# arrufat/zignal

Measured on NVIDIA H100. Metric: Mpixels/sec Gaussian-blur 8K RGBA f32, higher is better.
Workload: dtype f32

## Files before the change

### zignal_b200/csrc/zb_conv_fused.cu

```cuda
#include "zb_conv.h"
#include "zb_device.cuh"
#include "zb_shard.h"
#include "zb_tma.cuh"

namespace zb {

namespace {

constexpr int TW = 256;
constexpr int CHUNK = 8;
constexpr int G = TW / 8 + 2;
constexpr int STAGE_BYTES = G * CHUNK * 128;
constexpr int RING_ROWS = 24;
constexpr int RING_ROW_BYTES = TW * 16;
constexpr int RING_BYTES = RING_ROWS * RING_ROW_BYTES;
constexpr int NTHREADS = 256;
constexpr int MAX_HALF = 8;
constexpr int MAXK = 2 * MAX_HALF + 1;
constexpr int STAGES = 2;
constexpr int SMEM_BYTES = STAGES * STAGE_BYTES + RING_BYTES + 64 + 1024;

struct FusedParams {
    float kx[MAXK];
    float ky[MAXK];
    const float4* src;
    float4* dst;
    unsigned long long src_pitch_px, dst_pitch_px;
    int rows, cols, border;
    int ngroups;
    int n_strips;
    int n_units;
    int strip_lo, strip_hi;
    int n_segs, seg_chunks, seg_extra;
    int e_segs, e_chunks, e_extra;
    int row0, row1;
    int fix_rows;
    int fix_left;
    int fix_right;
    int tma_row_off;
    int edge_fast;
    int lsrc[8];
    int rsrc[8];
};

struct ShardParams {
    const float4* up_rows;
    const float4* down_rows;
    unsigned long long up_pitch_px, down_pitch_px;
    int half;
    ShardLink link;
};

template <bool ROTATE>
__device__ __forceinline__ void unit_at(const FusedParams& p, int u, int& strip, int& ra, int& rb) {
    const int n_inner = p.strip_hi - p.strip_lo;
    int seg, chunks, extra;
    if (u < p.n_segs * n_inner) {
        seg = u / n_inner;
        strip = p.strip_lo + (u - seg * n_inner);
        if constexpr (ROTATE) seg = seg + 1 == p.n_segs ? 0 : seg + 1;
        chunks = p.seg_chunks;
        extra = p.seg_extra;
    } else {
        const int n_edge = p.n_strips - n_inner;
        u -= p.n_segs * n_inner;
        seg = u / n_edge;
        const int e = u - seg * n_edge;
        strip = e < p.strip_lo ? e : e - p.strip_lo + p.strip_hi;
        chunks = p.e_chunks;
        extra = p.e_extra;
    }
    ra = p.row0 + (seg * chunks + min(seg, extra)) * CHUNK;
    rb = min(ra + (chunks + (seg < extra ? 1 : 0)) * CHUNK, p.row1);
}

template <bool EXACT>
__device__ __forceinline__ void mac4(float4& acc, const float4& v, float k) {
    if constexpr (EXACT) {
        acc.x = __fadd_rn(acc.x, __fmul_rn(v.x, k));
        acc.y = __fadd_rn(acc.y, __fmul_rn(v.y, k));
        acc.z = __fadd_rn(acc.z, __fmul_rn(v.z, k));
        acc.w = __fadd_rn(acc.w, __fmul_rn(v.w, k));
    } else {
        acc.x = fmaf(v.x, k, acc.x);
        acc.y = fmaf(v.y, k, acc.y);
        acc.z = fmaf(v.z, k, acc.z);
        acc.w = fmaf(v.w, k, acc.w);
    }
}

template <bool SHARD>
__device__ __noinline__ void fixup_stage(uint32_t stage, int y0, int xs0, bool fix_x, bool fix_rows, const FusedParams& p,
                                         int nb_lo, int nb_hi) {
    const int xlimit = p.ngroups * 8;
    auto stage_addr = [&](int rr, int xx) {
        const uint32_t line = (uint32_t)(rr * G + (xx >> 3));
        return stage + line * 128 + ((((uint32_t)xx & 7u) ^ (line & 7u)) << 4);
    };
    if (fix_x && p.edge_fast) {
        fix_x = false;
        if (threadIdx.x < 128) {
            const int side = threadIdx.x >> 6, rr = (threadIdx.x >> 3) & 7, e = threadIdx.x & 7;
            const int y = y0 + rr;
            bool row_ok = y >= 0 && y < p.rows;
            if constexpr (SHARD) row_ok = row_ok || (y < 0 && y >= nb_lo) || (y >= p.rows && y < nb_hi);
            const bool edge = side == 0 ? xs0 < 0 : xs0 + G * 8 > p.cols;
            if (row_ok && edge) {
                const int s_dst = side == 0 ? e : p.cols - xs0 + e;
                const int s_src = side == 0 ? p.lsrc[e] : p.rsrc[e] - xs0;
                if (s_dst < G * 8) sts128(stage_addr(rr, s_dst), lds128(stage_addr(rr, s_src)));
            }
        }
    }
    if (fix_x) {
        const int nleft = xs0 < 0 ? min(-xs0, G * 8) : 0;
        const int r0 = max(0, xlimit - xs0);
        const int r1 = min(G * 8, p.cols - xs0 + MAX_HALF);
        const int per_row = nleft + max(0, r1 - r0);
        for (int idx = threadIdx.x; idx < CHUNK * per_row; idx += NTHREADS) {
            const int rr = idx / per_row, e = idx - rr * per_row;
            const int xx = e < nleft ? e : r0 + (e - nleft);
            const int y = y0 + rr, x = xs0 + xx;
            const float4* rowp = p.src + (long long)y * (long long)p.src_pitch_px;
            if (y < 0 || y >= p.rows) {
                if constexpr (SHARD) {
                    if (y < nb_lo || y >= nb_hi) continue;
                } else {
                    continue;
                }
            }
            const int rx = resolve_index(x, p.cols, p.border);
            float4 v = make_float4(0.f, 0.f, 0.f, 0.f);
            if (rx >= 0) {
                const int sx = rx - xs0;
                if (rx < xlimit && sx >= 0 && sx < G * 8) v = lds128(stage_addr(rr, sx));
                else v = __ldg(rowp + rx);
            }
            sts128(stage_addr(rr, xx), v);
        }
    }
    if (fix_rows) {
        for (int idx = threadIdx.x; idx < CHUNK * G * 8; idx += NTHREADS) {
            const int rr = idx / (G * 8);
            const int xx = idx - rr * (G * 8);
            const int y = y0 + rr, x = xs0 + xx;
            if (y >= 0 && y < p.rows) continue;
            if constexpr (SHARD) {
                if (y >= nb_lo && y < nb_hi) continue;
            }
            const int ry = resolve_index(y, p.rows, p.border);
            const int rx = resolve_index(x, p.cols, p.border);
            float4 v = make_float4(0.f, 0.f, 0.f, 0.f);
            if (ry >= 0 && rx >= 0) v = __ldg(p.src + (size_t)ry * p.src_pitch_px + rx);
            sts128(stage_addr(rr, xx), v);
        }
    }
}

template <int HALF, bool EXACT, int SLOT>
__device__ __forceinline__ void v_pass(uint32_t v_col, const FusedParams& p, float4* out, bool col_ok, int rows_left) {
    constexpr int K = 2 * HALF + 1;
    constexpr int NLOAD = CHUNK + 2 * HALF;
    float4 acc[8];
#pragma unroll
    for (int o = 0; o < 8; ++o) acc[o] = make_float4(0.f, 0.f, 0.f, 0.f);
#pragma unroll
    for (int j = 0; j < NLOAD; ++j) {
        const int sr = (SLOT * CHUNK + 8 - HALF + j) % RING_ROWS;
        const float4 v = lds128(v_col + (uint32_t)(sr * RING_ROW_BYTES));
#pragma unroll
        for (int o = 0; o < 8; ++o) {
            const int ti = j - o;
            if (ti >= 0 && ti < K) mac4<EXACT>(acc[o], v, p.ky[ti]);
        }
    }
    if (col_ok) {
#pragma unroll
        for (int o = 0; o < 8; ++o)
            if (o < rows_left) __stcs(out + (size_t)o * p.dst_pitch_px, acc[o]);
    }
}

template <int HALF, bool EXACT, bool SHARD>
__device__ __forceinline__ uint32_t fused_units(const CUtensorMap& tmap, const FusedParams& p, unsigned nbr, int k_begin, int k_end, uint32_t count0) {
    constexpr int K = 2 * HALF + 1;
    constexpr int NLOAD = CHUNK + 2 * HALF;
    extern __shared__ unsigned char smem_raw[];
    const uint32_t smem0 = (smem_u32(smem_raw) + 1023u) & ~1023u;
    const uint32_t ring = smem0 + STAGES * STAGE_BYTES;
    const uint32_t bar0 = ring + RING_BYTES;

    const int tid = threadIdx.x;
    const long long u_first = (long long)blockIdx.x + (long long)k_begin * gridDim.x;
    const long long u_last = (long long)blockIdx.x + (long long)k_end * gridDim.x;
    const int n_units = (int)min((long long)p.n_units, u_last);
    if (u_first >= n_units) return count0;
    auto touches_neighbour = [&](int y) { return ((nbr & 1u) && y < 0) || ((nbr & 2u) && y + CHUNK > p.rows); };

    int pu = (int)u_first, pi = 0;
    uint32_t pcount = count0;
    auto produce = [&]() {
        if (pu >= n_units) return;
        int strip, ra, rb;
        unit_at<SHARD>(p, pu, strip, ra, rb);
        const int n_in = (rb - ra + CHUNK - 1) / CHUNK + 2;
        const uint32_t st = pcount % STAGES;
        const int y = ra - CHUNK + CHUNK * pi;
        fence_proxy_async();
        mbar_arrive_expect_tx(bar0 + 8 * st, STAGE_BYTES);
        tma_load_3d(smem0 + st * STAGE_BYTES, &tmap, 0, strip * (TW / 8) - 1, y + p.tma_row_off, bar0 + 8 * st);
        ++pcount;
        if (++pi == n_in) { pi = 0; pu += gridDim.x; }
    };
    if (tid == 0)
        for (int i = 0; i < STAGES; ++i) produce();

    const int ht = tid & 31, hr = tid >> 5;
    const int vx = tid;
    const uint32_t v_col = ring + (uint32_t)(vx >> 3) * 128u + ((((uint32_t)vx & 7u) ^ (((uint32_t)vx >> 3) & 7u)) << 4);
    const uint32_t h_ring_col = ring + (uint32_t)ht * 128u;
    const uint32_t h_key = (uint32_t)ht & 7u;

    uint32_t ccount = count0;

    for (int unit = (int)u_first; unit < n_units; unit += gridDim.x) {
        int strip, ra, rb;
        unit_at<SHARD>(p, unit, strip, ra, rb);
        const int x0 = strip * TW;
        const int n_out = (rb - ra + CHUNK - 1) / CHUNK;
        const int n_in = n_out + 2;
        const int g0 = x0 / 8 - 1;

        for (int i = 0; i < n_in; ++i, ++ccount) {
            const uint32_t st = ccount % STAGES;
            const uint32_t stage = smem0 + st * STAGE_BYTES;
            while (!mbar_try_wait(bar0 + 8 * st, (ccount / STAGES) & 1u)) {}
            const int y0 = ra - CHUNK + CHUNK * i;
            bool fix_r = p.fix_rows && (y0 < 0 || y0 + CHUNK > p.rows);
            if constexpr (SHARD) {
                if (touches_neighbour(y0)) fix_r = false;
            }
            const bool fix_x = (p.fix_left && g0 < 0) || (p.fix_right && (g0 + G) * 8 > p.ngroups * 8);
            if (fix_r || fix_x) {
                fixup_stage<SHARD>(stage, y0, g0 * 8, fix_x, fix_r, p, (nbr & 1u) ? INT_MIN : 0, (nbr & 2u) ? INT_MAX : p.rows);
                __syncthreads();
            }

            {
                const uint32_t line0 = (uint32_t)(hr * G + ht);
                uint32_t lbase[3];
#pragma unroll
                for (int l = 0; l < 3; ++l) lbase[l] = stage + (line0 + l) * 128u + (((line0 + l) & 7u) << 4);
                const uint32_t rrow = h_ring_col + (uint32_t)(((i % 3) * CHUNK + hr) * RING_ROW_BYTES);
                float4 acc[8];
#pragma unroll
                for (int o = 0; o < 8; ++o) acc[o] = make_float4(0.f, 0.f, 0.f, 0.f);
#pragma unroll
                for (int j = 0; j < NLOAD; ++j) {
                    const int pidx = 8 - HALF + j;
                    const float4 v = lds128(lbase[pidx >> 3] ^ (((uint32_t)pidx & 7u) << 4));
#pragma unroll
                    for (int o = 0; o < 8; ++o) {
                        const int ti = j - o;
                        if (ti >= 0 && ti < K) mac4<EXACT>(acc[o], v, p.kx[ti]);
                    }
                }
#pragma unroll
                for (int o = 0; o < 8; ++o) sts128(rrow + ((((uint32_t)o) ^ h_key) << 4), acc[o]);
            }
            __syncthreads();

            if (tid == 0) produce();

            if (i >= 2) {
                const int c = i - 2;
                const int x = x0 + vx;
                const int yb = ra + CHUNK * c;
                float4* out = p.dst + (size_t)yb * p.dst_pitch_px + x;
                const bool col_ok = x < p.cols;
                switch (c % 3) {
                    case 0: v_pass<HALF, EXACT, 0>(v_col, p, out, col_ok, rb - yb); break;
                    case 1: v_pass<HALF, EXACT, 1>(v_col, p, out, col_ok, rb - yb); break;
                    default: v_pass<HALF, EXACT, 2>(v_col, p, out, col_ok, rb - yb); break;
                }
            }
            __syncthreads();
        }
    }
    return ccount;
}

template <int HALF, bool EXACT, bool SHARD>
__device__ __forceinline__ void fused_sep_rgbaf32_body(const CUtensorMap& tmap, const FusedParams& p, const ShardParams* sp) {
    extern __shared__ unsigned char smem_raw[];
    const uint32_t smem0 = (smem_u32(smem_raw) + 1023u) & ~1023u;
    const uint32_t bar0 = smem0 + STAGES * STAGE_BYTES + RING_BYTES;
    const int tid = threadIdx.x;
    if (tid == 0) {
        asm volatile("prefetch.tensormap [%0];" ::"l"(&tmap) : "memory");
        for (int i = 0; i < STAGES; ++i) mbar_init(bar0 + 8 * i, 1);
        fence_barrier_init();
    }
    if constexpr (!SHARD) {
        __syncthreads();
        fused_units<HALF, EXACT, false>(tmap, p, 0u, 0, INT_MAX / 2048, 0u);
    } else {
        ShardCtrl* me = sp->link.self;
        const unsigned long long epoch = sp->link.epoch;
        const unsigned nbr = (sp->up_rows ? 1u : 0u) | (sp->down_rows ? 2u : 0u);
        const int per_side = sp->half * p.cols;
        const int total = (sp->up_rows ? per_side : 0) + (sp->down_rows ? per_side : 0);
        constexpr int BATCH = 12;
        const int rem = p.n_units % (int)gridDim.x;
        const int n_copiers = (int)gridDim.x - rem;
        const int ci = (int)blockIdx.x - rem;
        const bool copier = ci >= 0 && (long long)ci * NTHREADS * BATCH < total;
        if (tid == 0) {
            if (blockIdx.x == 0) {
                me->dbg[0] = global_timer_ns();
                if (sp->link.up) st_release_sys(&sp->link.up->ready_from[1], epoch);
                if (sp->link.down) st_release_sys(&sp->link.down->ready_from[0], epoch);
            }
            if (copier) {
                if (sp->up_rows) shard_wait_ge(&me->ready_from[0], epoch, me);
                if (sp->down_rows) shard_wait_ge(&me->ready_from[1], epoch, me);
                if (ci == 0) me->dbg[1] = global_timer_ns();
            }
        }
        __syncthreads();
        if (copier) {
            for (int base = ci * NTHREADS * BATCH; base < total; base += n_copiers * NTHREADS * BATCH) {
                float4 v[BATCH];
                float4* dstp[BATCH];
    #pragma unroll
                for (int k = 0; k < BATCH; ++k) {
                    int e = base + k * NTHREADS + tid;
                    dstp[k] = nullptr;
                    if (e < total) {
                        const bool upper = sp->up_rows && e < per_side;
                        if (!upper && sp->up_rows) e -= per_side;
                        const int r = e / p.cols, x = e - r * p.cols;
                        if (upper) {
                            v[k] = *(sp->up_rows + (size_t)r * sp->up_pitch_px + x);
                            dstp[k] = const_cast<float4*>(p.src) + (long long)(r - sp->half) * (long long)p.src_pitch_px + x;
                        } else {
                            v[k] = *(sp->down_rows + (size_t)r * sp->down_pitch_px + x);
                            dstp[k] = const_cast<float4*>(p.src) + (long long)(p.rows + r) * (long long)p.src_pitch_px + x;
                        }
                    }
                }
    #pragma unroll
                for (int k = 0; k < BATCH; ++k)
                    if (dstp[k]) *dstp[k] = v[k];
            }
            asm volatile("fence.proxy.async;" ::: "memory");
            __syncthreads();
        }
        if (tid == 0) {
            __threadfence();
            if (atomicAdd(&me->halo_reads[0], 1u) == gridDim.x - 1u) {
                me->halo_reads[0] = 0;
                me->dbg[2] = global_timer_ns();
                __threadfence();
                st_release_sys(&me->halo_landed, epoch);
                if (sp->up_rows) st_release_sys(&sp->link.up->done_from[1], epoch);
                if (sp->down_rows) st_release_sys(&sp->link.down->done_from[0], epoch);
            }
        }
        const long long first_halo_unit = (long long)max(0, p.n_segs - 2) * p.n_strips;
        const int k_split = first_halo_unit <= (long long)blockIdx.x ? 0 : (int)((first_halo_unit - blockIdx.x + gridDim.x - 1) / gridDim.x);
        const uint32_t count = fused_units<HALF, EXACT, true>(tmap, p, nbr, 0, k_split, 0u);
        if ((long long)blockIdx.x + (long long)k_split * gridDim.x < (long long)p.n_units) {
            if (tid == 0) {
                shard_wait_ge(&me->halo_landed, epoch, me);
                asm volatile("fence.proxy.async;" ::: "memory");
            }
            __syncthreads();
            fused_units<HALF, EXACT, true>(tmap, p, nbr, k_split, INT_MAX / 2048, count);
        }
        if (tid == 0) {
            ShardCtrl* me = sp->link.self;
            __threadfence();
            if (atomicAdd(&me->exit_ticket, 1u) == gridDim.x - 1u) {
                me->exit_ticket = 0;
                me->dbg[3] = global_timer_ns();
                if (sp->link.up) shard_wait_ge(&me->done_from[0], sp->link.epoch, me);
                if (sp->link.down) shard_wait_ge(&me->done_from[1], sp->link.epoch, me);
                me->dbg[4] = global_timer_ns();
            }
        }
    }
}


template <int HALF, bool EXACT>
__global__ void __launch_bounds__(NTHREADS, 1)
fused_sep_rgbaf32_kernel(const __grid_constant__ CUtensorMap tmap, const __grid_constant__ FusedParams p) {
    fused_sep_rgbaf32_body<HALF, EXACT, false>(tmap, p, nullptr);
}

template <int HALF, bool EXACT>
__global__ void __launch_bounds__(NTHREADS, 1)
fused_sep_rgbaf32_shard_kernel(const __grid_constant__ CUtensorMap tmap, const __grid_constant__ FusedParams p,
                               const __grid_constant__ ShardParams sp) {
    fused_sep_rgbaf32_body<HALF, EXACT, true>(tmap, p, &sp);
}

template <int HALF>
int launch_fused(const CUtensorMap& tmap, const FusedParams& p, const ShardParams* sp, int grid, bool exact, cudaStream_t s) {
    if (sp) {
        auto k = exact ? fused_sep_rgbaf32_shard_kernel<HALF, true> : fused_sep_rgbaf32_shard_kernel<HALF, false>;
        ZB_CUDA(cudaFuncSetAttribute(k, cudaFuncAttributeMaxDynamicSharedMemorySize, SMEM_BYTES));
        k<<<grid, NTHREADS, SMEM_BYTES, s>>>(tmap, p, *sp);
    } else {
        auto k = exact ? fused_sep_rgbaf32_kernel<HALF, true> : fused_sep_rgbaf32_kernel<HALF, false>;
        ZB_CUDA(cudaFuncSetAttribute(k, cudaFuncAttributeMaxDynamicSharedMemorySize, SMEM_BYTES));
        k<<<grid, NTHREADS, SMEM_BYTES, s>>>(tmap, p);
    }
    ZB_LAUNCHED();
    return ZB_OK;
}

int launch_half(int half, const CUtensorMap& tmap, const FusedParams& p, const ShardParams* sp, int grid, bool exact, cudaStream_t s) {
    switch (half) {
        case 1: return launch_fused<1>(tmap, p, sp, grid, exact, s);
        case 2: return launch_fused<2>(tmap, p, sp, grid, exact, s);
        case 3: return launch_fused<3>(tmap, p, sp, grid, exact, s);
        case 4: return launch_fused<4>(tmap, p, sp, grid, exact, s);
        case 5: return launch_fused<5>(tmap, p, sp, grid, exact, s);
        case 6: return launch_fused<6>(tmap, p, sp, grid, exact, s);
        case 7: return launch_fused<7>(tmap, p, sp, grid, exact, s);
        case 8: return launch_fused<8>(tmap, p, sp, grid, exact, s);
    }
    return ZB_ERR_UNSUPPORTED;
}

}

static int encode_block_map(EncodeTiledFn encode, CUtensorMap& tmap, void* data, int ngroups, int rows, uint64_t stride_px) {
    const cuuint64_t gdim[3] = {32, (cuuint64_t)ngroups, (cuuint64_t)rows};
    const cuuint64_t gstr[2] = {128, (cuuint64_t)stride_px * 16};
    const cuuint32_t box[3] = {32, (cuuint32_t)G, (cuuint32_t)CHUNK};
    const cuuint32_t estr[3] = {1, 1, 1};
    CUresult cr = encode(&tmap, CU_TENSOR_MAP_DATA_TYPE_FLOAT32, 3, data, gdim, gstr, box, estr, CU_TENSOR_MAP_INTERLEAVE_NONE,
                         CU_TENSOR_MAP_SWIZZLE_128B, CU_TENSOR_MAP_L2_PROMOTION_L2_256B, CU_TENSOR_MAP_FLOAT_OOB_FILL_NONE);
    if (cr != CUDA_SUCCESS) {
        snprintf(t_last_error, sizeof(t_last_error), "cuTensorMapEncodeTiled failed: %d", (int)cr);
        return ZB_ERR_UNSUPPORTED;
    }
    return ZB_OK;
}

constexpr long long EDGE_COST_NUM = 5, EDGE_COST_DEN = 4;

static void plan_units(int nrows, int sm_count, FusedParams& p) {
    const long long chunks = (nrows + CHUNK - 1) / CHUNK;
    const long long max_segs = chunks / 8 < 1 ? 1 : (chunks / 8 < sm_count ? chunks / 8 : sm_count);
    const long long n_inner = p.strip_hi - p.strip_lo, n_edge = p.n_strips - n_inner;
    auto steps = [&](long long segs) { return (chunks + segs - 1) / segs + 2; };
    long long best_cost = -1, best_units = 0, best_s = 1, best_e = 1;
    for (long long s = 1; s <= max_segs; ++s) {
        const long long waves = (s * p.n_strips + sm_count - 1) / sm_count;
        long long e = s;
        if (n_edge > 0) {
            long long e_max = (waves * sm_count - s * n_inner) / n_edge;
            if (e_max > max_segs) e_max = max_segs;
            while (e < e_max && EDGE_COST_NUM * steps(e) > EDGE_COST_DEN * steps(s)) ++e;
        }
        const long long inner = n_inner > 0 ? EDGE_COST_DEN * steps(s) : 0, edge = n_edge > 0 ? EDGE_COST_NUM * steps(e) : 0;
        const long long cost = waves * (inner > edge ? inner : edge), units = s * n_inner + e * n_edge;
        if (best_cost < 0 || cost < best_cost || (cost == best_cost && units < best_units)) {
            best_cost = cost;
            best_units = units;
            best_s = s;
            best_e = e;
        }
    }
    p.n_units = (int)best_units;
    p.n_segs = (int)best_s;
    p.seg_chunks = (int)(chunks / best_s);
    p.seg_extra = (int)(chunks % best_s);
    p.e_segs = (int)best_e;
    p.e_chunks = (int)(chunks / best_e);
    p.e_extra = (int)(chunks % best_e);
}

static int fused_prepare(const zb_image* src, zb_image* dst, const float* kx, int nx, const float* ky, int ny, int border, int row0, int row1,
                         bool bands, FusedParams& p, CUtensorMap& tmap, int& grid, int& half_out, EncodeTiledFn& encode) {
    const int half_x = nx / 2, half_y = ny / 2;
    const int half = half_x > half_y ? half_x : half_y;
    if (half < 1 || half > MAX_HALF) return ZB_ERR_UNSUPPORTED;
    if (src->cols < 16 || src->rows < 16) return ZB_ERR_UNSUPPORTED;
    if (images_overlap(src, dst, 16)) return ZB_ERR_UNSUPPORTED;
    if (((uintptr_t)src->data & 15u) || ((uintptr_t)dst->data & 15u)) return ZB_ERR_UNSUPPORTED;
    for (int i = 0; i < nx; ++i) if (fabsf(kx[i]) < 1e-10f) return ZB_ERR_UNSUPPORTED;
    for (int i = 0; i < ny; ++i) if (fabsf(ky[i]) < 1e-10f) return ZB_ERR_UNSUPPORTED;
    encode = encode_tiled_fn();
    if (!encode) return ZB_ERR_UNSUPPORTED;
    DeviceInfo di;
    int rc = device_info(&di);
    if (rc) return rc;
    if (di.smem_optin < (size_t)SMEM_BYTES) return ZB_ERR_UNSUPPORTED;

    memset(&p, 0, sizeof(p));
    for (int i = 0; i < nx; ++i) p.kx[i + (half - half_x)] = kx[i];
    for (int i = 0; i < ny; ++i) p.ky[i + (half - half_y)] = ky[i];
    p.src = (const float4*)src->data;
    p.dst = (float4*)dst->data;
    p.src_pitch_px = src->stride;
    p.dst_pitch_px = dst->stride;
    p.rows = (int)src->rows;
    p.cols = (int)src->cols;
    p.border = border;
    p.ngroups = p.cols / 8;
    p.n_strips = (p.cols + TW - 1) / TW;
    p.row0 = row0 < 0 ? 0 : row0;
    p.row1 = (row1 < 0 || row1 > p.rows) ? p.rows : row1;
    if (p.row1 <= p.row0) { grid = 0; return ZB_OK; }
    const int nrows = p.row1 - p.row0;
    p.fix_rows = border != ZB_BORDER_ZERO;
    p.fix_left = border != ZB_BORDER_ZERO;
    p.fix_right = (border != ZB_BORDER_ZERO) || (p.cols % 8 != 0);
    p.strip_lo = 0;
    p.strip_hi = p.n_strips;
    if (bands) {
        const int band_target = g_tune_band_rows.load();
        int n_bands = (nrows + band_target - 1) / band_target;
        const long long waves = ((long long)n_bands * p.n_strips + di.sm_count - 1) / di.sm_count;
        int nb2 = (int)((waves * di.sm_count) / p.n_strips);
        if (nb2 > n_bands) n_bands = nb2;
        int band_rows = (nrows + n_bands - 1) / n_bands;
        band_rows = ((band_rows + CHUNK - 1) / CHUNK) * CHUNK;
        if (band_rows < 64) band_rows = 64;
        p.n_segs = (nrows + band_rows - 1) / band_rows;
        p.seg_chunks = band_rows / CHUNK;
        p.n_units = p.n_segs * p.n_strips;
    } else {
        if (p.fix_left) p.strip_lo = 1;
        while (p.fix_right && p.strip_hi > p.strip_lo && (p.strip_hi - 1) * (TW / 8) - 1 + G > p.ngroups) --p.strip_hi;
        if (p.strip_hi <= p.strip_lo) { p.strip_lo = 0; p.strip_hi = p.n_strips; }
        plan_units(nrows, di.sm_count, p);
    }
    p.edge_fast = g_tune_edge_fast.load() && (border == ZB_BORDER_REPLICATE || border == ZB_BORDER_MIRROR) && p.cols % 8 == 0 && p.cols >= 16;
    for (int e = 0; e < 8; ++e) {
        const int xl = e - 8, xr = p.cols + e;
        p.lsrc[e] = 8 + (border == ZB_BORDER_REPLICATE ? 0 : -xl);
        p.rsrc[e] = border == ZB_BORDER_REPLICATE ? p.cols - 1 : 2 * (p.cols - 1) - xr;
    }

    if ((rc = encode_block_map(encode, tmap, src->data, p.ngroups, p.rows, src->stride))) return rc;
    grid = p.n_units < di.sm_count ? p.n_units : di.sm_count;
    half_out = half;
    return ZB_OK;
}

int conv_separable_fused_rgbaf32(const zb_image* src, zb_image* dst, const float* kx, int nx, const float* ky, int ny, int border,
                                 bool exact, cudaStream_t s, int row0, int row1) {
    FusedParams p;
    CUtensorMap tmap;
    EncodeTiledFn encode;
    int grid = 0, half = 0;
    int rc = fused_prepare(src, dst, kx, nx, ky, ny, border, row0, row1, false, p, tmap, grid, half, encode);
    if (rc || grid == 0) return rc;
    t_last_kernel = exact ? "fused_sep_rgbaf32_exact" : "fused_sep_rgbaf32";
    return launch_half(half, tmap, p, nullptr, grid, exact, s);
}

int conv_separable_fused_rgbaf32_shard(const zb_image* src, zb_image* dst, const float* kx, int nx, const float* ky, int ny, int border,
                                       bool exact, const PeerBlock& up, const PeerBlock& down, uint32_t halo_cap, const ShardLink& link,
                                       cudaStream_t s) {
    if (src->rows % CHUNK != 0 || halo_cap < (uint32_t)CHUNK) return ZB_ERR_UNSUPPORTED;
    FusedParams p;
    CUtensorMap tmap;
    EncodeTiledFn encode;
    int grid = 0, half = 0;
    int rc = fused_prepare(src, dst, kx, nx, ky, ny, border, 0, -1, true, p, tmap, grid, half, encode);
    if (rc) return rc;
    if (grid == 0) return ZB_ERR_UNSUPPORTED;
    const uint32_t hv = (uint32_t)(ny / 2);
    if ((up.data && (up.rows < hv || ((uintptr_t)up.data & 15u))) || (down.data && (down.rows < hv || ((uintptr_t)down.data & 15u))))
        return ZB_ERR_UNSUPPORTED;
    void* ext = (char*)src->data - (size_t)halo_cap * src->stride * 16;
    if ((rc = encode_block_map(encode, tmap, ext, p.ngroups, (int)(src->rows + 2 * halo_cap), src->stride))) return rc;
    p.tma_row_off = (int)halo_cap;
    p.fix_rows = 1;
    ShardParams sp;
    memset(&sp, 0, sizeof(sp));
    sp.half = (int)hv;
    if (up.data && hv) {
        sp.up_rows = (const float4*)up.data + (size_t)(up.rows - hv) * up.stride;
        sp.up_pitch_px = up.stride;
    }
    if (down.data && hv) {
        sp.down_rows = (const float4*)down.data;
        sp.down_pitch_px = down.stride;
    }
    sp.link = link;
    if (!sp.up_rows) sp.link.up = nullptr;
    if (!sp.down_rows) sp.link.down = nullptr;
    {
        DeviceInfo di;
        if ((rc = device_info(&di))) return rc;
        grid = di.sm_count;
    }
    t_last_kernel = exact ? "fused_sep_rgbaf32_shard_exact" : "fused_sep_rgbaf32_shard";
    return launch_half(half, tmap, p, &sp, grid, exact, s);
}

}
```

### zignal_b200/csrc/zb_tma.cuh

```cuda
#pragma once
#include <cuda.h>
#include <cuda_runtime.h>

#include <cstdint>

namespace zb {

__device__ __forceinline__ uint32_t smem_u32(const void* p) { return (uint32_t)__cvta_generic_to_shared(p); }
__device__ __forceinline__ float4 lds128(uint32_t addr) {
    float4 v;
    asm volatile("ld.shared.v4.f32 {%0, %1, %2, %3}, [%4];" : "=f"(v.x), "=f"(v.y), "=f"(v.z), "=f"(v.w) : "r"(addr));
    return v;
}
__device__ __forceinline__ void sts128(uint32_t addr, const float4& v) {
    asm volatile("st.shared.v4.f32 [%0], {%1, %2, %3, %4};" ::"r"(addr), "f"(v.x), "f"(v.y), "f"(v.z), "f"(v.w) : "memory");
}
__device__ __forceinline__ void mbar_init(uint32_t bar, uint32_t count) {
    asm volatile("mbarrier.init.shared::cta.b64 [%0], %1;" ::"r"(bar), "r"(count) : "memory");
}
__device__ __forceinline__ void fence_barrier_init() { asm volatile("fence.mbarrier_init.release.cluster;" ::: "memory"); }
__device__ __forceinline__ void fence_proxy_async() { asm volatile("fence.proxy.async.shared::cta;" ::: "memory"); }
__device__ __forceinline__ void mbar_arrive_expect_tx(uint32_t bar, uint32_t bytes) {
    asm volatile("mbarrier.arrive.expect_tx.shared::cta.b64 _, [%0], %1;" ::"r"(bar), "r"(bytes) : "memory");
}
__device__ __forceinline__ bool mbar_try_wait(uint32_t bar, uint32_t parity) {
    uint32_t ok;
    asm volatile(
        "{\n\t.reg .pred p;\n\t"
        "mbarrier.try_wait.parity.shared::cta.b64 p, [%1], %2;\n\t"
        "selp.u32 %0, 1, 0, p;\n\t}"
        : "=r"(ok)
        : "r"(bar), "r"(parity)
        : "memory");
    return ok != 0;
}
__device__ __forceinline__ void tma_load_3d(uint32_t dst, const CUtensorMap* tmap, int c0, int c1, int c2, uint32_t bar) {
    asm volatile(
        "cp.async.bulk.tensor.3d.shared::cluster.global.tile.mbarrier::complete_tx::bytes [%0], [%1, {%2, %3, %4}], [%5];" ::"r"(dst),
        "l"(tmap), "r"(c0), "r"(c1), "r"(c2), "r"(bar)
        : "memory");
}


__device__ __forceinline__ void tma_load_2d(uint32_t dst, const CUtensorMap* tmap, int c0, int c1, uint32_t bar) {
    asm volatile("cp.async.bulk.tensor.2d.shared::cluster.global.tile.mbarrier::complete_tx::bytes [%0], [%1, {%2, %3}], [%4];" ::"r"(dst),
                 "l"(tmap), "r"(c0), "r"(c1), "r"(bar)
                 : "memory");
}
__device__ __forceinline__ int4 lds128_i(uint32_t addr) {
    int4 v;
    asm volatile("ld.shared.v4.s32 {%0, %1, %2, %3}, [%4];" : "=r"(v.x), "=r"(v.y), "=r"(v.z), "=r"(v.w) : "r"(addr));
    return v;
}
__device__ __forceinline__ void sts128_i(uint32_t addr, const int4& v) {
    asm volatile("st.shared.v4.s32 [%0], {%1, %2, %3, %4};" ::"r"(addr), "r"(v.x), "r"(v.y), "r"(v.z), "r"(v.w) : "memory");
}
__device__ __forceinline__ uint32_t lds32(uint32_t addr) {
    uint32_t v;
    asm volatile("ld.shared.u32 %0, [%1];" : "=r"(v) : "r"(addr));
    return v;
}
__device__ __forceinline__ void sts32(uint32_t addr, uint32_t v) { asm volatile("st.shared.u32 [%0], %1;" ::"r"(addr), "r"(v) : "memory"); }

}
```

Baseline: 85360.

## Write fused blur output via TMA bulk tensor stores from a shared tile

In the non-sharded fused separable blur, each vertical-pass result is staged into a new shared-memory output tile and written to global memory by one thread issuing a TMA 3D store with an L2 evict-first hint. Per-thread streaming stores remain only for columns beyond the TMA-covered region. The aim is to offload global writes to the async copy engine and overlap them with the next chunk's compute. The cost is a larger shared-memory footprint, an extra proxy fence, and a wait on the previous bulk store before the tile is reused each iteration.

```diff
diff --git a/zignal_b200/csrc/zb_conv_fused.cu b/zignal_b200/csrc/zb_conv_fused.cu
--- a/zignal_b200/csrc/zb_conv_fused.cu
+++ b/zignal_b200/csrc/zb_conv_fused.cu
@@ -18,7 +18,8 @@
 constexpr int MAX_HALF = 8;
 constexpr int MAXK = 2 * MAX_HALF + 1;
 constexpr int STAGES = 2;
-constexpr int SMEM_BYTES = STAGES * STAGE_BYTES + RING_BYTES + 64 + 1024;
+constexpr int OTILE_BYTES = CHUNK * TW * 16;
+constexpr int SMEM_BYTES = STAGES * STAGE_BYTES + RING_BYTES + OTILE_BYTES + 64 + 1024;
 
 struct FusedParams {
     float kx[MAXK];
@@ -157,8 +158,8 @@
     }
 }
 
-template <int HALF, bool EXACT, int SLOT>
-__device__ __forceinline__ void v_pass(uint32_t v_col, const FusedParams& p, float4* out, bool col_ok, int rows_left) {
+template <int HALF, bool EXACT, int SLOT, bool SHARD>
+__device__ __forceinline__ void v_pass(uint32_t v_col, const FusedParams& p, uint32_t o_px, float4* out, bool direct, int rows_left) {
     constexpr int K = 2 * HALF + 1;
     constexpr int NLOAD = CHUNK + 2 * HALF;
     float4 acc[8];
@@ -174,7 +175,11 @@
             if (ti >= 0 && ti < K) mac4<EXACT>(acc[o], v, p.ky[ti]);
         }
     }
-    if (col_ok) {
+    if constexpr (!SHARD) {
+#pragma unroll
+        for (int o = 0; o < 8; ++o) sts128(o_px + (uint32_t)(o * TW * 16), acc[o]);
+    }
+    if (direct) {
 #pragma unroll
         for (int o = 0; o < 8; ++o)
             if (o < rows_left) __stcs(out + (size_t)o * p.dst_pitch_px, acc[o]);
@@ -182,13 +187,15 @@
 }
 
 template <int HALF, bool EXACT, bool SHARD>
-__device__ __forceinline__ uint32_t fused_units(const CUtensorMap& tmap, const FusedParams& p, unsigned nbr, int k_begin, int k_end, uint32_t count0) {
+__device__ __forceinline__ uint32_t fused_units(const CUtensorMap& tmap, const CUtensorMap* dmap, const FusedParams& p, unsigned nbr, int k_begin,
+                                                int k_end, uint32_t count0) {
     constexpr int K = 2 * HALF + 1;
     constexpr int NLOAD = CHUNK + 2 * HALF;
     extern __shared__ unsigned char smem_raw[];
     const uint32_t smem0 = (smem_u32(smem_raw) + 1023u) & ~1023u;
     const uint32_t ring = smem0 + STAGES * STAGE_BYTES;
-    const uint32_t bar0 = ring + RING_BYTES;
+    const uint32_t otile = ring + RING_BYTES;
+    const uint32_t bar0 = otile + OTILE_BYTES;
 
     const int tid = threadIdx.x;
     const long long u_first = (long long)blockIdx.x + (long long)k_begin * gridDim.x;
@@ -218,6 +225,7 @@
     const int ht = tid & 31, hr = tid >> 5;
     const int vx = tid;
     const uint32_t v_col = ring + (uint32_t)(vx >> 3) * 128u + ((((uint32_t)vx & 7u) ^ (((uint32_t)vx >> 3) & 7u)) << 4);
+    const uint32_t o_px = otile + (uint32_t)vx * 16u;
     const uint32_t h_ring_col = ring + (uint32_t)ht * 128u;
     const uint32_t h_key = (uint32_t)ht & 7u;
 
@@ -268,6 +276,9 @@
 #pragma unroll
                 for (int o = 0; o < 8; ++o) sts128(rrow + ((((uint32_t)o) ^ h_key) << 4), acc[o]);
             }
+            if constexpr (!SHARD) {
+                if (tid == 0) bulk_wait_group_read0();
+            }
             __syncthreads();
 
             if (tid == 0) produce();
@@ -277,33 +288,43 @@
                 const int x = x0 + vx;
                 const int yb = ra + CHUNK * c;
                 float4* out = p.dst + (size_t)yb * p.dst_pitch_px + x;
-                const bool col_ok = x < p.cols;
+                const bool direct = x < p.cols && (SHARD || x >= p.ngroups * 8);
                 switch (c % 3) {
-                    case 0: v_pass<HALF, EXACT, 0>(v_col, p, out, col_ok, rb - yb); break;
-                    case 1: v_pass<HALF, EXACT, 1>(v_col, p, out, col_ok, rb - yb); break;
-                    default: v_pass<HALF, EXACT, 2>(v_col, p, out, col_ok, rb - yb); break;
+                    case 0: v_pass<HALF, EXACT, 0, SHARD>(v_col, p, o_px, out, direct, rb - yb); break;
+                    case 1: v_pass<HALF, EXACT, 1, SHARD>(v_col, p, o_px, out, direct, rb - yb); break;
+                    default: v_pass<HALF, EXACT, 2, SHARD>(v_col, p, o_px, out, direct, rb - yb); break;
                 }
+                if constexpr (!SHARD) fence_proxy_async();
             }
             __syncthreads();
+            if constexpr (!SHARD) {
+                if (tid == 0 && i >= 2) {
+                    tma_store_3d(dmap, otile, 0, x0 / 8, ra + CHUNK * (i - 2), l2_evict_first_policy());
+                    bulk_commit_group();
+                }
+            }
         }
     }
     return ccount;
 }
 
 template <int HALF, bool EXACT, bool SHARD>
-__device__ __forceinline__ void fused_sep_rgbaf32_body(const CUtensorMap& tmap, const FusedParams& p, const ShardParams* sp) {
+__device__ __forceinline__ void fused_sep_rgbaf32_body(const CUtensorMap& tmap, const CUtensorMap* dmap, const FusedParams& p,
+                                                       const ShardParams* sp) {
     extern __shared__ unsigned char smem_raw[];
     const uint32_t smem0 = (smem_u32(smem_raw) + 1023u) & ~1023u;
-    const uint32_t bar0 = smem0 + STAGES * STAGE_BYTES + RING_BYTES;
+    const uint32_t bar0 = smem0 + STAGES * STAGE_BYTES + RING_BYTES + OTILE_BYTES;
     const int tid = threadIdx.x;
     if (tid == 0) {
         asm volatile("prefetch.tensormap [%0];" ::"l"(&tmap) : "memory");
+        if constexpr (!SHARD) asm volatile("prefetch.tensormap [%0];" ::"l"(dmap) : "memory");
         for (int i = 0; i < STAGES; ++i) mbar_init(bar0 + 8 * i, 1);
         fence_barrier_init();
     }
     if constexpr (!SHARD) {
         __syncthreads();
-        fused_units<HALF, EXACT, false>(tmap, p, 0u, 0, INT_MAX / 2048, 0u);
+        fused_units<HALF, EXACT, false>(tmap, dmap, p, 0u, 0, INT_MAX / 2048, 0u);
+        if (tid == 0) bulk_wait_group_read0();
     } else {
         ShardCtrl* me = sp->link.self;
         const unsigned long long epoch = sp->link.epoch;
@@ -369,14 +390,14 @@
         }
         const long long first_halo_unit = (long long)max(0, p.n_segs - 2) * p.n_strips;
         const int k_split = first_halo_unit <= (long long)blockIdx.x ? 0 : (int)((first_halo_unit - blockIdx.x + gridDim.x - 1) / gridDim.x);
-        const uint32_t count = fused_units<HALF, EXACT, true>(tmap, p, nbr, 0, k_split, 0u);
+        const uint32_t count = fused_units<HALF, EXACT, true>(tmap, nullptr, p, nbr, 0, k_split, 0u);
         if ((long long)blockIdx.x + (long long)k_split * gridDim.x < (long long)p.n_units) {
             if (tid == 0) {
                 shard_wait_ge(&me->halo_landed, epoch, me);
                 asm volatile("fence.proxy.async;" ::: "memory");
             }
             __syncthreads();
-            fused_units<HALF, EXACT, true>(tmap, p, nbr, k_split, INT_MAX / 2048, count);
+            fused_units<HALF, EXACT, true>(tmap, nullptr, p, nbr, k_split, INT_MAX / 2048, count);
         }
         if (tid == 0) {
             ShardCtrl* me = sp->link.self;
@@ -395,19 +416,21 @@
 
 template <int HALF, bool EXACT>
 __global__ void __launch_bounds__(NTHREADS, 1)
-fused_sep_rgbaf32_kernel(const __grid_constant__ CUtensorMap tmap, const __grid_constant__ FusedParams p) {
-    fused_sep_rgbaf32_body<HALF, EXACT, false>(tmap, p, nullptr);
+fused_sep_rgbaf32_kernel(const __grid_constant__ CUtensorMap tmap, const __grid_constant__ FusedParams p,
+                         const __grid_constant__ CUtensorMap dmap) {
+    fused_sep_rgbaf32_body<HALF, EXACT, false>(tmap, &dmap, p, nullptr);
 }
 
 template <int HALF, bool EXACT>
 __global__ void __launch_bounds__(NTHREADS, 1)
 fused_sep_rgbaf32_shard_kernel(const __grid_constant__ CUtensorMap tmap, const __grid_constant__ FusedParams p,
                                const __grid_constant__ ShardParams sp) {
-    fused_sep_rgbaf32_body<HALF, EXACT, true>(tmap, p, &sp);
+    fused_sep_rgbaf32_body<HALF, EXACT, true>(tmap, nullptr, p, &sp);
 }
 
 template <int HALF>
-int launch_fused(const CUtensorMap& tmap, const FusedParams& p, const ShardParams* sp, int grid, bool exact, cudaStream_t s) {
+int launch_fused(const CUtensorMap& tmap, const CUtensorMap* dmap, const FusedParams& p, const ShardParams* sp, int grid, bool exact,
+                 cudaStream_t s) {
     if (sp) {
         auto k = exact ? fused_sep_rgbaf32_shard_kernel<HALF, true> : fused_sep_rgbaf32_shard_kernel<HALF, false>;
         ZB_CUDA(cudaFuncSetAttribute(k, cudaFuncAttributeMaxDynamicSharedMemorySize, SMEM_BYTES));
@@ -415,35 +438,37 @@
     } else {
         auto k = exact ? fused_sep_rgbaf32_kernel<HALF, true> : fused_sep_rgbaf32_kernel<HALF, false>;
         ZB_CUDA(cudaFuncSetAttribute(k, cudaFuncAttributeMaxDynamicSharedMemorySize, SMEM_BYTES));
-        k<<<grid, NTHREADS, SMEM_BYTES, s>>>(tmap, p);
+        k<<<grid, NTHREADS, SMEM_BYTES, s>>>(tmap, p, *dmap);
     }
     ZB_LAUNCHED();
     return ZB_OK;
 }
 
-int launch_half(int half, const CUtensorMap& tmap, const FusedParams& p, const ShardParams* sp, int grid, bool exact, cudaStream_t s) {
+int launch_half(int half, const CUtensorMap& tmap, const CUtensorMap* dmap, const FusedParams& p, const ShardParams* sp, int grid, bool exact,
+                cudaStream_t s) {
     switch (half) {
-        case 1: return launch_fused<1>(tmap, p, sp, grid, exact, s);
-        case 2: return launch_fused<2>(tmap, p, sp, grid, exact, s);
-        case 3: return launch_fused<3>(tmap, p, sp, grid, exact, s);
-        case 4: return launch_fused<4>(tmap, p, sp, grid, exact, s);
-        case 5: return launch_fused<5>(tmap, p, sp, grid, exact, s);
-        case 6: return launch_fused<6>(tmap, p, sp, grid, exact, s);
-        case 7: return launch_fused<7>(tmap, p, sp, grid, exact, s);
-        case 8: return launch_fused<8>(tmap, p, sp, grid, exact, s);
+        case 1: return launch_fused<1>(tmap, dmap, p, sp, grid, exact, s);
+        case 2: return launch_fused<2>(tmap, dmap, p, sp, grid, exact, s);
+        case 3: return launch_fused<3>(tmap, dmap, p, sp, grid, exact, s);
+        case 4: return launch_fused<4>(tmap, dmap, p, sp, grid, exact, s);
+        case 5: return launch_fused<5>(tmap, dmap, p, sp, grid, exact, s);
+        case 6: return launch_fused<6>(tmap, dmap, p, sp, grid, exact, s);
+        case 7: return launch_fused<7>(tmap, dmap, p, sp, grid, exact, s);
+        case 8: return launch_fused<8>(tmap, dmap, p, sp, grid, exact, s);
     }
     return ZB_ERR_UNSUPPORTED;
 }
 
 }
 
-static int encode_block_map(EncodeTiledFn encode, CUtensorMap& tmap, void* data, int ngroups, int rows, uint64_t stride_px) {
+static int encode_block_map(EncodeTiledFn encode, CUtensorMap& tmap, void* data, int ngroups, int rows, uint64_t stride_px, int box_groups,
+                            CUtensorMapSwizzle swizzle) {
     const cuuint64_t gdim[3] = {32, (cuuint64_t)ngroups, (cuuint64_t)rows};
     const cuuint64_t gstr[2] = {128, (cuuint64_t)stride_px * 16};
-    const cuuint32_t box[3] = {32, (cuuint32_t)G, (cuuint32_t)CHUNK};
+    const cuuint32_t box[3] = {32, (cuuint32_t)box_groups, (cuuint32_t)CHUNK};
     const cuuint32_t estr[3] = {1, 1, 1};
     CUresult cr = encode(&tmap, CU_TENSOR_MAP_DATA_TYPE_FLOAT32, 3, data, gdim, gstr, box, estr, CU_TENSOR_MAP_INTERLEAVE_NONE,
-                         CU_TENSOR_MAP_SWIZZLE_128B, CU_TENSOR_MAP_L2_PROMOTION_L2_256B, CU_TENSOR_MAP_FLOAT_OOB_FILL_NONE);
+                         swizzle, CU_TENSOR_MAP_L2_PROMOTION_L2_256B, CU_TENSOR_MAP_FLOAT_OOB_FILL_NONE);
     if (cr != CUDA_SUCCESS) {
         snprintf(t_last_error, sizeof(t_last_error), "cuTensorMapEncodeTiled failed: %d", (int)cr);
         return ZB_ERR_UNSUPPORTED;
@@ -548,7 +573,7 @@
         p.rsrc[e] = border == ZB_BORDER_REPLICATE ? p.cols - 1 : 2 * (p.cols - 1) - xr;
     }
 
-    if ((rc = encode_block_map(encode, tmap, src->data, p.ngroups, p.rows, src->stride))) return rc;
+    if ((rc = encode_block_map(encode, tmap, src->data, p.ngroups, p.rows, src->stride, G, CU_TENSOR_MAP_SWIZZLE_128B))) return rc;
     grid = p.n_units < di.sm_count ? p.n_units : di.sm_count;
     half_out = half;
     return ZB_OK;
@@ -562,8 +587,10 @@
     int grid = 0, half = 0;
     int rc = fused_prepare(src, dst, kx, nx, ky, ny, border, row0, row1, false, p, tmap, grid, half, encode);
     if (rc || grid == 0) return rc;
+    CUtensorMap dmap;
+    if ((rc = encode_block_map(encode, dmap, dst->data, p.ngroups, p.row1, dst->stride, TW / 8, CU_TENSOR_MAP_SWIZZLE_NONE))) return rc;
     t_last_kernel = exact ? "fused_sep_rgbaf32_exact" : "fused_sep_rgbaf32";
-    return launch_half(half, tmap, p, nullptr, grid, exact, s);
+    return launch_half(half, tmap, &dmap, p, nullptr, grid, exact, s);
 }
 
 int conv_separable_fused_rgbaf32_shard(const zb_image* src, zb_image* dst, const float* kx, int nx, const float* ky, int ny, int border,
@@ -581,7 +608,8 @@
     if ((up.data && (up.rows < hv || ((uintptr_t)up.data & 15u))) || (down.data && (down.rows < hv || ((uintptr_t)down.data & 15u))))
         return ZB_ERR_UNSUPPORTED;
     void* ext = (char*)src->data - (size_t)halo_cap * src->stride * 16;
-    if ((rc = encode_block_map(encode, tmap, ext, p.ngroups, (int)(src->rows + 2 * halo_cap), src->stride))) return rc;
+    if ((rc = encode_block_map(encode, tmap, ext, p.ngroups, (int)(src->rows + 2 * halo_cap), src->stride, G, CU_TENSOR_MAP_SWIZZLE_128B)))
+        return rc;
     p.tma_row_off = (int)halo_cap;
     p.fix_rows = 1;
     ShardParams sp;
@@ -604,7 +632,7 @@
         grid = di.sm_count;
     }
     t_last_kernel = exact ? "fused_sep_rgbaf32_shard_exact" : "fused_sep_rgbaf32_shard";
-    return launch_half(half, tmap, p, &sp, grid, exact, s);
-}
-
-}
+    return launch_half(half, tmap, nullptr, p, &sp, grid, exact, s);
+}
+
+}
diff --git a/zignal_b200/csrc/zb_tma.cuh b/zignal_b200/csrc/zb_tma.cuh
--- a/zignal_b200/csrc/zb_tma.cuh
+++ b/zignal_b200/csrc/zb_tma.cuh
@@ -40,7 +40,18 @@
         "l"(tmap), "r"(c0), "r"(c1), "r"(c2), "r"(bar)
         : "memory");
 }
-
+__device__ __forceinline__ uint64_t l2_evict_first_policy() {
+    uint64_t pol;
+    asm volatile("createpolicy.fractional.L2::evict_first.b64 %0, 1.0;" : "=l"(pol));
+    return pol;
+}
+__device__ __forceinline__ void tma_store_3d(const CUtensorMap* tmap, uint32_t src, int c0, int c1, int c2, uint64_t policy) {
+    asm volatile("cp.async.bulk.tensor.3d.global.shared::cta.bulk_group.L2::cache_hint [%0, {%1, %2, %3}], [%4], %5;" ::"l"(tmap),
+                 "r"(c0), "r"(c1), "r"(c2), "r"(src), "l"(policy)
+                 : "memory");
+}
+__device__ __forceinline__ void bulk_commit_group() { asm volatile("cp.async.bulk.commit_group;" ::: "memory"); }
+__device__ __forceinline__ void bulk_wait_group_read0() { asm volatile("cp.async.bulk.wait_group.read 0;" ::: "memory"); }
 
 __device__ __forceinline__ void tma_load_2d(uint32_t dst, const CUtensorMap* tmap, int c0, int c1, uint32_t bar) {
     asm volatile("cp.async.bulk.tensor.2d.shared::cluster.global.tile.mbarrier::complete_tx::bytes [%0], [%1, {%2, %3}], [%4];" ::"r"(dst),
```

Result: no change. 85940, median of 6 (+0.7%).
